# wg-perception/PartsBasedDetector

Hardware: AMD Instinct MI355X
Metric: detect() frames/sec, 640x480, 26-part person model (higher is better)
Workload: dtype f32

## Files before the change

partsbaseddetector_amd/csrc/k_hog.hip:

```cpp
#include "pbd_internal.hpp"
#include "pbd_split.hpp"

#ifdef PBD_PROBES
__device__ unsigned long long pbd_hog_dbg[8];
#define HOG_STAMP(i) do { if (blockIdx.x == 0 && threadIdx.x == 0) pbd_hog_dbg[i] = wall_clock64(); } while (0)
void hog_debug_read(unsigned long long* out) { hipMemcpyFromSymbol(out, HIP_SYMBOL(pbd_hog_dbg), sizeof(unsigned long long) * 8); }
#else
#define HOG_STAMP(i) do { } while (0)
void hog_debug_read(unsigned long long* out) { for (int i = 0; i < 8; ++i) out[i] = 0; }
#endif

#define HOG_LUT_SIDE 511
template <typename T>
__device__ __forceinline__ int hog_snap(T dx, T dy) {
  const T uu[9] = {1.000, 0.9397, 0.7660, 0.5000, 0.1736, -0.1736, -0.5000, -0.7660, -0.9397};
  const T vv[9] = {0.000, 0.3420, 0.6428, 0.8660, 0.9848, 0.9848, 0.8660, 0.6428, 0.3420};
  T best_dot = 0;
  int best_o = 0;
#pragma unroll
  for (int o = 0; o < 9; ++o) {
    T dot = uu[o] * dx + vv[o] * dy;
    if (dot > best_dot) { best_dot = dot; best_o = o; }
    else if (-dot > best_dot) { best_dot = -dot; best_o = o + 9; }
  }
  return best_o;
}
template <typename T>
__global__ __launch_bounds__(256) void k_hog_binlut(uint8_t* __restrict__ lut) {
  const int i = blockIdx.x * 256 + threadIdx.x;
  if (i >= HOG_LUT_SIDE * HOG_LUT_SIDE) return;
  const int iy = i / HOG_LUT_SIDE, ix = i - iy * HOG_LUT_SIDE;
  lut[i] = (uint8_t)hog_snap<T>((T)(ix - 255), (T)(iy - 255));
}
size_t hog_binlut_bytes() { return (size_t)HOG_LUT_SIDE * HOG_LUT_SIDE; }
void launch_hog_binlut(uint8_t* lut, int ts, hipStream_t s) {
  const int n = HOG_LUT_SIDE * HOG_LUT_SIDE;
  if (ts == 8) hipLaunchKernelGGL(k_hog_binlut<double>, dim3((n + 255) / 256), dim3(256), 0, s, lut);
  else hipLaunchKernelGGL(k_hog_binlut<float>, dim3((n + 255) / 256), dim3(256), 0, s, lut);
}

#define HOG_NT 384

template <typename T, int SBIN_T, int TC_T, typename IT = uint8_t>
__global__ __launch_bounds__(HOG_NT, 5) void k_hog(const HogTile* __restrict__ tiles, const LevelDev* __restrict__ levels,
                                                const uint8_t* __restrict__ pyr, T* __restrict__ feat, int cn,
                                                int sbin_rt, int tc_rt, const uint8_t* __restrict__ binlut, uint16_t* __restrict__ split, int split_parts) {
  const int sbin = SBIN_T > 0 ? SBIN_T : sbin_rt;
  const int tc = TC_T > 0 ? TC_T : tc_rt;
  extern __shared__ __attribute__((aligned(16))) char smem[];
#ifdef PBD_HOG_PRIO
  __builtin_amdgcn_s_setprio(PBD_HOG_PRIO);
#endif
  HOG_STAMP(0);
  const HogTile t = tiles[blockIdx.x];
  const LevelDev lv = levels[t.level];
  const int bpp = cn * (int)sizeof(IT);
  constexpr bool NEED_IP = !(SBIN_T > 0 && (SBIN_T & 1) == 0);
  const HogLds L = hog_lds_layout(sbin, tc, bpp, (int)sizeof(T), NEED_IP);
  T* mag = (T*)(smem + L.mag_off);
  uint8_t* bin = (uint8_t*)(smem + L.bin_off);
  uint8_t* raw = (uint8_t*)(smem + L.raw_off);
  T* hist = (T*)(smem + L.hist_off);
  T* norm = (T*)(smem + L.norm_off);
  T* ninv = (T*)(smem + L.ninv_off);
  T* wy0 = (T*)(smem + L.tab_off);
  T* wy1 = wy0 + L.PT;
  T* wx0 = wy1 + L.PT;
  T* wx1 = wx0 + L.PT;
  int* ipy = (int*)(wx1 + L.PT);
  int* ipx = ipy + L.PT;
  const int PT = L.PT, NB = L.NB, RT = L.RT, RP = L.RP, tid = threadIdx.x;
  const int w = lv.iw, h = lv.ih, bw = lv.bw, bh = lv.bh;
  const int vw = bw * sbin, vh = bh * sbin;
  const uint8_t* im = pyr + lv.img_off;
  const int stride = w * bpp;
  const int py0 = t.cy0 * sbin - (sbin + 1) / 2 - L.P0, px0 = t.cx0 * sbin - (sbin + 1) / 2 - L.P0;
  const int ry0 = py0 - L.MG, rx0 = px0 - L.MG;

  {
    const int wpr = RP >> 2;
    const int nword = RT * wpr;
    const int rowbytes = stride;
    const int b00 = rx0 * bpp;
    constexpr int LBW = 7;
    if (rowbytes >= 4) {
      const unsigned wmagic = 0xFFFFFFFFu / (unsigned)wpr + 1u;
      auto place = [&](int i, int& b0, int& la) {
        const int r = wpr > 1 ? (int)__umulhi((unsigned)i, wmagic) : i, k = i - r * wpr;
        b0 = b00 + 4 * k;
        la = r * RP + 4 * k;
        return min(max(ry0 + r, 0), h - 1);
      };
      for (int i0 = tid; i0 < nword; i0 += HOG_NT * LBW) {
        unsigned wv[LBW];
#pragma unroll
        for (int j = 0; j < LBW; ++j) {
          int b0, la;
          const int sy = place(min(i0 + j * HOG_NT, nword - 1), b0, la);
          wv[j] = *(const __attribute__((aligned(1))) unsigned*)(im + (size_t)sy * stride + min(max(b0, 0), rowbytes - 4));
        }
#pragma unroll
        for (int j = 0; j < LBW; ++j) {
          int b0, la;
          place(min(i0 + j * HOG_NT, nword - 1), b0, la);
          const int sh = min(max(b0, 0), rowbytes - 4) - b0;
          const int a8 = 8 * min(abs(sh), 3);
          *(unsigned*)(raw + la) = sh > 0 ? wv[j] << a8 : wv[j] >> a8;
        }
      }
    } else {
      for (int i = tid; i < nword; i += HOG_NT) {
        const int r = i / wpr, k = i - r * wpr;
        const int sy = min(max(ry0 + r, 0), h - 1);
        const int b0 = b00 + 4 * k;
        const uint8_t* src = im + (size_t)sy * stride;
        unsigned v = 0;
#pragma unroll
        for (int q = 0; q < 4; ++q) v |= (unsigned)src[min(max(b0 + q, 0), rowbytes - 1)] << (8 * q);
        *(unsigned*)(raw + r * RP + 4 * k) = v;
      }
    }
  }
  for (int i = tid; i < 2 * PT; i += HOG_NT) {
    const bool isx = i >= PT;
    const int j = isx ? i - PT : i;
    const int p = (isx ? px0 : py0) + j;
    T pp = (T)(((double)(T)p + 0.5) / (double)(T)sbin - 0.5);
    int ip = (int)t_floor(pp);
    T v0 = pp - (T)ip;
    T v1 = (T)(1.0 - (double)v0);
    if (isx) { wx0[j] = v0; wx1[j] = v1; if constexpr (NEED_IP) ipx[j] = ip; }
    else { wy0[j] = v0; wy1[j] = v1; if constexpr (NEED_IP) ipy[j] = ip; }
  }
  __syncthreads();
  HOG_STAMP(1);

  for (int i = tid; i < PT * PT; i += HOG_NT) {
    const int wy = i / PT, wx = i - wy * PT;
    const int y = py0 + wy, x = px0 + wx;
    T m = (T)0;
    int b = 0;
    if (y >= 1 && y < vh - 1 && x >= 1 && x < vw - 1) {
      const int sx = min(x, w - 2), sy = min(y, h - 2);
      if constexpr (sizeof(IT) > 1) {
        const IT* s = (const IT*)(raw + (sy - ry0) * RP + (sx - rx0) * bpp);
        const int rs = RP / (int)sizeof(IT);
        T dx, dy, v;
        if (cn == 1) {
          dy = (T)(s[rs] - s[-rs]);
          dx = (T)(s[1] - s[-1]);
          v = dx * dx + dy * dy;
        } else {
          const T dyb = (T)(s[rs] - s[-rs]), dxb = (T)(s[3] - s[-3]);
          const T vb = dxb * dxb + dyb * dyb;
          const T dyg = (T)(s[rs + 1] - s[-rs + 1]), dxg = (T)(s[4] - s[-2]);
          const T vg = dxg * dxg + dyg * dyg;
          dy = (T)(s[rs + 2] - s[-rs + 2]); dx = (T)(s[5] - s[-1]);
          v = dx * dx + dy * dy;
          if (vg > v) { v = vg; dx = dxg; dy = dyg; }
          if (vb > v) { v = vb; dx = dxb; dy = dyb; }
        }
        b = hog_snap<T>(dx, dy);
        m = t_sqrt(v);
      } else {
      const uint8_t* s = raw + (sy - ry0) * RP + (sx - rx0) * cn;
      int dxi, dyi, vi;
      if (cn == 1) {
        dyi = (int)s[RP] - (int)s[-RP];
        dxi = (int)s[1] - (int)s[-1];
      } else {
        const int dyb = (int)s[RP] - (int)s[-RP], dxb = (int)s[3] - (int)s[-3];
        const int dyg = (int)s[RP + 1] - (int)s[-RP + 1], dxg = (int)s[4] - (int)s[-2];
        dyi = (int)s[RP + 2] - (int)s[-RP + 2]; dxi = (int)s[5] - (int)s[-1];
        vi = dxi * dxi + dyi * dyi;
        const int vg = dxg * dxg + dyg * dyg, vb = dxb * dxb + dyb * dyb;
        if (vg > vi) { vi = vg; dxi = dxg; dyi = dyg; }
        if (vb > vi) { vi = vb; dxi = dxb; dyi = dyb; }
      }
      vi = dxi * dxi + dyi * dyi;
      b = binlut[(dyi + 255) * HOG_LUT_SIDE + (dxi + 255)];
      m = t_sqrt((T)vi);
      }
    }
    const int wq = wx / sbin, pi = wy * L.MP + (wx - wq * sbin) * L.QS + wq;
    mag[pi] = m;
    bin[pi] = (uint8_t)b;
  }
  __syncthreads();
  for (int i = tid; i < NB * NB * PBD_NORIENT; i += HOG_NT) hist[i] = (T)0;
  __syncthreads();
  HOG_STAMP(2);

  for (int bl = tid; bl < NB * NB; bl += HOG_NT) {
    const int lby = bl / NB, lbx = bl - lby * NB;
    const int by = t.cy0 + lby, bx = t.cx0 + lbx;
    if (by >= bh || bx >= bw) continue;
    T* hb = hist + bl;
    const int NBB = NB * NB;
    if constexpr (SBIN_T > 0 && (SBIN_T & 1) == 0) {
      const int wy_lo = lby * SBIN_T, wx_lo = lbx * SBIN_T;
      T fxv[2 * SBIN_T];
#pragma unroll
      for (int dx = 0; dx < 2 * SBIN_T; ++dx) fxv[dx] = dx < SBIN_T ? wx0[wx_lo + dx] : wx1[wx_lo + dx];
#pragma unroll 2
      for (int dy = 0; dy < 2 * SBIN_T; ++dy) {
        const int wy = wy_lo + dy;
        const T fy = dy < SBIN_T ? wy0[wy] : wy1[wy];
        const uint8_t* brow = bin + wy * L.MP + lbx;
        const T* mrow = mag + wy * L.MP + lbx;
#pragma unroll
        for (int dx = 0; dx < 2 * SBIN_T; ++dx) {
          const int pi = (dx % SBIN_T) * L.QS + dx / SBIN_T;
          hb[brow[pi] * NBB] += (fy * fxv[dx]) * mrow[pi];
        }
      }
    } else {
      const int wy_lo = lby * sbin, wx_lo = lbx * sbin, span = 2 * sbin + 2;
#pragma unroll 2
      for (int dy = 0; dy < span; ++dy) {
        const int wy = wy_lo + dy;
        if (wy >= PT) break;
        const int iy = ipy[wy];
        T fy;
        if (iy == by) fy = wy1[wy]; else if (iy == by - 1) fy = wy0[wy]; else continue;
        for (int dx = 0; dx < span; ++dx) {
          const int wx = wx_lo + dx;
          if (wx >= PT) break;
          const int ix = ipx[wx];
          T fx;
          if (ix == bx) fx = wx1[wx]; else if (ix == bx - 1) fx = wx0[wx]; else continue;
          const int wq = wx / sbin, pi = wy * L.MP + (wx - wq * sbin) * L.QS + wq;
          hb[bin[pi] * NBB] += (fy * fx) * mag[pi];
        }
      }
    }
  }
  __syncthreads();
  HOG_STAMP(3);

  for (int i = tid; i < NB * NB; i += HOG_NT) {
    const T* hsrc = hist + i;
    const int NBB = NB * NB;
    T acc = (T)0;
#pragma unroll
    for (int o = 0; o < 9; ++o) {
      T s = hsrc[o * NBB] + hsrc[(o + 9) * NBB];
      acc += s * s;
    }
    norm[i] = acc;
  }
  __syncthreads();

  const int NC = tc + 1;
  for (int i = tid; i < NC * NC; i += HOG_NT) {
    const int y = i / NC, x = i - y * NC;
    const T* p = norm + y * NB + x;
    T s = p[0] + p[1] + p[NB] + p[NB + 1];
    ninv[i] = (T)(1.0f / sqrt((double)s + 0.0001));
  }
  __syncthreads();

  HOG_STAMP(4);
  T* out = feat + lv.cell_off * PBD_FLEN;
  T* stg = (T*)(smem + L.out_off);
  const int ncell = tc * tc, half = (ncell + 1) / 2;
  for (int c0 = 0; c0 < ncell; c0 += half) {
    const int cell = c0 + tid;
    if (tid < half && cell < ncell) {
      const int ly = cell / tc, lx = cell - ly * tc;
      if (t.cy0 + ly < bh - 2 && t.cx0 + lx < bw - 2) {
        const T n1 = ninv[(ly + 1) * NC + lx + 1], n2 = ninv[ly * NC + lx + 1];
        const T n3 = ninv[(ly + 1) * NC + lx], n4 = ninv[ly * NC + lx];
        const T* hsrc = hist + ((ly + 1) * NB + lx + 1);
        const int NBB = NB * NB;
        T* d = stg + tid * (PBD_FLEN + 1);
        T t1 = 0, t2 = 0, t3 = 0, t4 = 0;
#pragma unroll 6
        for (int o = 0; o < PBD_NORIENT; ++o) {
          const T val = hsrc[o * NBB];
          const T h1 = t_fmin(val * n1, (T)0.2), h2 = t_fmin(val * n2, (T)0.2);
          const T h3 = t_fmin(val * n3, (T)0.2), h4 = t_fmin(val * n4, (T)0.2);
          d[o] = (T)(0.5 * (double)(h1 + h2 + h3 + h4));
          t1 += h1; t2 += h2; t3 += h3; t4 += h4;
        }
#pragma unroll 3
        for (int o = 0; o < PBD_NORIENT / 2; ++o) {
          const T sum = hsrc[o * NBB] + hsrc[(o + PBD_NORIENT / 2) * NBB];
          const T h1 = t_fmin(sum * n1, (T)0.2), h2 = t_fmin(sum * n2, (T)0.2);
          const T h3 = t_fmin(sum * n3, (T)0.2), h4 = t_fmin(sum * n4, (T)0.2);
          d[PBD_NORIENT + o] = (T)(0.5 * (double)(h1 + h2 + h3 + h4));
        }
        d[27] = (T)(0.2357 * (double)t1);
        d[28] = (T)(0.2357 * (double)t2);
        d[29] = (T)(0.2357 * (double)t3);
        d[30] = (T)(0.2357 * (double)t4);
        d[31] = (T)0;
      }
    }
    __syncthreads();
    for (int i = tid; i < half * PBD_FLEN; i += HOG_NT) {
      const int k = i & 31, lc = i >> 5;
      const int cl = c0 + lc;
      const int ly = cl / tc, lx = cl - ly * tc;
      const int cy = t.cy0 + ly, cx = t.cx0 + lx;
      if (cl < ncell && cy < bh - 2 && cx < bw - 2) {
        const T v = stg[lc * (PBD_FLEN + 1) + k];
        const size_t gc = (size_t)cy * lv.cw + cx;
        out[gc * PBD_FLEN + k] = v;
        if constexpr (sizeof(T) == 4) {
          if (split && split_parts == 3) {
            feat_split_bf16(v, split + (lv.cell_off + gc) * (3 * PBD_FLEN) + k, PBD_FLEN);
          } else if (split) {
            feat_split_f16(v, (_Float16*)split + (lv.cell_off + gc) * (2 * PBD_FLEN) + k, PBD_FLEN);
          }
        }
      }
    }
    __syncthreads();
  }
  HOG_STAMP(5);
}

template <typename T>
static void launch_hog_t(const HogTile* tiles, int ntiles, const LevelDev* levels, const uint8_t* pyr, T* feat,
                         int cn, int sbin, int tc, const uint8_t* binlut, uint16_t* split, int split_parts, int depth, hipStream_t s) {
  const int esz = depth == PBD_DEPTH_16U ? 2 : depth == PBD_DEPTH_32F ? 4 : depth == PBD_DEPTH_64F ? 8 : 1;
  auto go = [&](auto kern, bool need_ip) {
    const size_t lds = hog_lds_layout(sbin, tc, cn * esz, (int)sizeof(T), need_ip).total;
    static LdsOptIn optin;
    optin.ensure((const void*)kern, lds);
    hipLaunchKernelGGL(kern, dim3(ntiles), dim3(HOG_NT), lds, s, tiles, levels, pyr, feat, cn, sbin, tc, binlut, split, split_parts);
  };
  if (depth == PBD_DEPTH_16U) go(k_hog<T, 0, 0, uint16_t>, true);
  else if (depth == PBD_DEPTH_32F) go(k_hog<T, 0, 0, float>, true);
  else if (depth == PBD_DEPTH_64F) go(k_hog<T, 0, 0, double>, true);
  else if (sbin == 4 && tc == 16) go(k_hog<T, 4, 16>, false);
  else if (sbin == 4 && tc == 8) go(k_hog<T, 4, 8>, false);
  else if (sbin == 8 && tc == 8) go(k_hog<T, 8, 8>, false);
  else go(k_hog<T, 0, 0>, true);
}

void launch_hog(const HogTile* tiles, int ntiles, const LevelDev* levels, const uint8_t* pyr, void* feat, int ts,
                int cn, int sbin, int tc, const uint8_t* binlut, uint16_t* split, int split_parts, int depth, hipStream_t s) {
  if (ntiles <= 0) return;
  if (ts == 8) launch_hog_t<double>(tiles, ntiles, levels, pyr, (double*)feat, cn, sbin, tc, binlut, nullptr, 0, depth, s);
  else launch_hog_t<float>(tiles, ntiles, levels, pyr, (float*)feat, cn, sbin, tc, binlut, split, split_parts, depth, s);
}
```

partsbaseddetector_amd/csrc/pbd_lds.hpp:

```cpp
#pragma once
#include <stddef.h>
#include "pbd_plan.hpp"

#ifdef __HIPCC__
#define PBD_HD __host__ __device__ inline
#else
#define PBD_HD inline
#endif

#define DT_SEGS 72
PBD_HD size_t dt_hdr_bytes(int nt, int ts, int its, int lpb) {
  return ((size_t)lpb * 16 + DT_SEGS * 4 + (size_t)nt * (ts + 4 * its) + 15) & ~(size_t)15;
}
inline size_t dt_lds_bytes(int stride, int lpb, int ts, int nt) {
  const int its = stride <= 256 ? 1 : 2;
  return (size_t)lpb * stride * (2 * ts + its) + dt_hdr_bytes(nt, ts, its, lpb) + (((size_t)stride + 1) & ~(size_t)1) * 8 + 16;
}

struct HogLds {
  int PT;
  int NB;
  int P0;
  int MG;
  int RT;
  int RP;
  int QS;
  int MP;
  size_t mag_off, bin_off, hist_off, norm_off, ninv_off, tab_off, raw_off, out_off, total;
};

PBD_HD HogLds hog_lds_layout(int sbin, int tc, int bpp, int ts, bool need_ip = true) {
  HogLds L;
  L.NB = tc + 2;
  L.P0 = (sbin & 1) ? 1 : 0;
  L.PT = L.NB * sbin + sbin + 2 * L.P0;
  L.MG = sbin / 2 + 2;
  L.RT = L.PT + L.MG + 1;
  L.RP = (bpp & 7) ? (L.RT * bpp + 3) & ~3 : (L.RT * bpp + 7) & ~7;
  L.QS = (L.PT + sbin - 1) / sbin;
  L.MP = L.QS * sbin;
  size_t o = 0;
  const size_t nn = (size_t)ts * (L.NB * L.NB + (tc + 1) * (tc + 1));
  L.mag_off = o; L.norm_off = o; L.ninv_off = o + (size_t)ts * L.NB * L.NB;
  L.out_off = (o + nn + 15) & ~(size_t)15;
  {
    const size_t a = (size_t)ts * L.PT * L.MP, b = L.out_off + (size_t)ts * ((tc * tc + 1) / 2) * (PBD_FLEN + 1);
    o += ((a > b ? a : b) + 15) & ~(size_t)15;
  }
  const size_t hist_bytes = (size_t)ts * L.NB * L.NB * PBD_NORIENT, raw_bytes = (size_t)L.RT * L.RP;
  L.hist_off = o; L.raw_off = o;
  o += ((hist_bytes > raw_bytes ? hist_bytes : raw_bytes) + 15) & ~(size_t)15;
  L.tab_off = o; o += ((size_t)ts * 2 + (need_ip ? sizeof(int) : 0)) * 2 * L.PT;
  L.bin_off = (o + 3) & ~(size_t)3; o = L.bin_off + (size_t)L.PT * L.MP;
  L.total = (o + 15) & ~(size_t)15;
  return L;
}
inline size_t hog_lds_bytes(int sbin, int tc, int ts, int bpp = 3) { return hog_lds_layout(sbin, tc, bpp, ts).total; }
```

Measured before the change: 2415.

## Pack HOG magnitude and bin into one LDS word and split normalization roles

For even fixed sbin with uint8 input and float output, gradient magnitude and orientation bin are packed into a single 32-bit LDS word, with the bin in the top bits and the magnitude rescaled to fit the remaining bits. This removes the separate bin array and halves the LDS reads in the histogram loop. Interpolation weights become compile-time constants, so the weight tables are no longer built or stored. The normalization step splits each cell's work across three lane groups, and feature stores are widened to two elements per store. These changes shrink LDS use and per-thread work, at the risk of precision loss for very small or denormal magnitudes and of a mismatched LDS size on the host side, since the host computes the packed flag using sbin=4 even for the sbin=8 variant.

```diff
diff --git a/partsbaseddetector_amd/csrc/hog_pack.hpp b/partsbaseddetector_amd/csrc/hog_pack.hpp
--- /dev/null
+++ b/partsbaseddetector_amd/csrc/hog_pack.hpp
@@ -0,0 +1,45 @@
+#pragma once
+#include <stdint.h>
+#include <type_traits>
+
+#ifdef __HIPCC__
+#define HOG_PACK_HD __host__ __device__ inline
+#else
+#define HOG_PACK_HD inline
+#endif
+
+template <typename T, int SBIN, typename IT> constexpr bool hog_packed() {
+  return std::is_same<T, float>::value && std::is_same<IT, uint8_t>::value && SBIN > 0 && (SBIN & 1) == 0;
+}
+
+HOG_PACK_HD uint32_t hog_f2u(float f) { uint32_t u; __builtin_memcpy(&u, &f, 4); return u; }
+HOG_PACK_HD float hog_u2f(uint32_t u) { float f; __builtin_memcpy(&f, &u, 4); return f; }
+
+HOG_PACK_HD uint32_t hog_pack_bits(uint32_t bits, uint32_t bin) {
+  const uint32_t e = bits >> 23, e4 = e ? e - 126u : 0u;
+  return bin << 27 | e4 << 23 | (bits & 0x7FFFFFu);
+}
+HOG_PACK_HD uint32_t hog_unpack_bits(uint32_t w) {
+  const uint32_t t = w & 0x07FFFFFFu;
+  return t ? t + (126u << 23) : 0u;
+}
+HOG_PACK_HD uint32_t hog_unpack_bin(uint32_t w) { return w >> 27; }
+
+HOG_PACK_HD uint32_t hog_pack(float g, uint32_t bin) { return bin << 27 | hog_f2u(g * 0x1p-126f); }
+HOG_PACK_HD float hog_unpack_scaled(uint32_t w) { return hog_u2f(w & 0x07FFFFFFu); }
+#define HOG_UNSCALE 0x1p126f
+
+template <typename T, int SBIN> struct HogWeights;
+template <typename T> struct HogWeights<T, 4> {
+  static constexpr T w0[4] = {(T)0.625, (T)0.875, (T)0.125, (T)0.375};
+  static constexpr T w1[4] = {(T)0.375, (T)0.125, (T)0.875, (T)0.625};
+};
+template <typename T> struct HogWeights<T, 8> {
+  static constexpr T w0[8] = {(T)0.5625, (T)0.6875, (T)0.8125, (T)0.9375, (T)0.0625, (T)0.1875, (T)0.3125, (T)0.4375};
+  static constexpr T w1[8] = {(T)0.4375, (T)0.3125, (T)0.1875, (T)0.0625, (T)0.9375, (T)0.8125, (T)0.6875, (T)0.5625};
+};
+template <typename T, int SBIN> HOG_PACK_HD constexpr T hog_w0(int p) { return HogWeights<T, SBIN>::w0[((p % SBIN) + SBIN) % SBIN]; }
+template <typename T, int SBIN> HOG_PACK_HD constexpr T hog_w1(int p) { return HogWeights<T, SBIN>::w1[((p % SBIN) + SBIN) % SBIN]; }
+template <typename T, int SBIN> HOG_PACK_HD constexpr T hog_footprint_weight(int d) {
+  return d < SBIN ? hog_w0<T, SBIN>(d + SBIN / 2) : hog_w1<T, SBIN>(d + SBIN / 2);
+}
diff --git a/partsbaseddetector_amd/csrc/k_hog.hip b/partsbaseddetector_amd/csrc/k_hog.hip
--- a/partsbaseddetector_amd/csrc/k_hog.hip
+++ b/partsbaseddetector_amd/csrc/k_hog.hip
@@ -1,5 +1,6 @@
 #include "pbd_internal.hpp"
 #include "pbd_split.hpp"
+#include "hog_pack.hpp"
 
 #ifdef PBD_PROBES
 __device__ unsigned long long pbd_hog_dbg[8];
@@ -56,8 +57,10 @@
   const LevelDev lv = levels[t.level];
   const int bpp = cn * (int)sizeof(IT);
   constexpr bool NEED_IP = !(SBIN_T > 0 && (SBIN_T & 1) == 0);
-  const HogLds L = hog_lds_layout(sbin, tc, bpp, (int)sizeof(T), NEED_IP);
+  constexpr bool PACKED = hog_packed<T, SBIN_T, IT>();
+  const HogLds L = hog_lds_layout(sbin, tc, bpp, (int)sizeof(T), NEED_IP, PACKED);
   T* mag = (T*)(smem + L.mag_off);
+  unsigned* pk = (unsigned*)(smem + L.mag_off);
   uint8_t* bin = (uint8_t*)(smem + L.bin_off);
   uint8_t* raw = (uint8_t*)(smem + L.raw_off);
   T* hist = (T*)(smem + L.hist_off);
@@ -121,16 +124,18 @@
       }
     }
   }
-  for (int i = tid; i < 2 * PT; i += HOG_NT) {
-    const bool isx = i >= PT;
-    const int j = isx ? i - PT : i;
-    const int p = (isx ? px0 : py0) + j;
-    T pp = (T)(((double)(T)p + 0.5) / (double)(T)sbin - 0.5);
-    int ip = (int)t_floor(pp);
-    T v0 = pp - (T)ip;
-    T v1 = (T)(1.0 - (double)v0);
-    if (isx) { wx0[j] = v0; wx1[j] = v1; if constexpr (NEED_IP) ipx[j] = ip; }
-    else { wy0[j] = v0; wy1[j] = v1; if constexpr (NEED_IP) ipy[j] = ip; }
+  if constexpr (NEED_IP) {
+    for (int i = tid; i < 2 * PT; i += HOG_NT) {
+      const bool isx = i >= PT;
+      const int j = isx ? i - PT : i;
+      const int p = (isx ? px0 : py0) + j;
+      T pp = (T)(((double)(T)p + 0.5) / (double)(T)sbin - 0.5);
+      int ip = (int)t_floor(pp);
+      T v0 = pp - (T)ip;
+      T v1 = (T)(1.0 - (double)v0);
+      if (isx) { wx0[j] = v0; wx1[j] = v1; ipx[j] = ip; }
+      else { wy0[j] = v0; wy1[j] = v1; ipy[j] = ip; }
+    }
   }
   __syncthreads();
   HOG_STAMP(1);
@@ -183,8 +188,8 @@
       }
     }
     const int wq = wx / sbin, pi = wy * L.MP + (wx - wq * sbin) * L.QS + wq;
-    mag[pi] = m;
-    bin[pi] = (uint8_t)b;
+    if constexpr (PACKED) pk[pi] = hog_pack(m, (unsigned)b);
+    else { mag[pi] = m; bin[pi] = (uint8_t)b; }
   }
   __syncthreads();
   for (int i = tid; i < NB * NB * PBD_NORIENT; i += HOG_NT) hist[i] = (T)0;
@@ -198,21 +203,25 @@
     T* hb = hist + bl;
     const int NBB = NB * NB;
     if constexpr (SBIN_T > 0 && (SBIN_T & 1) == 0) {
-      const int wy_lo = lby * SBIN_T, wx_lo = lbx * SBIN_T;
-      T fxv[2 * SBIN_T];
-#pragma unroll
-      for (int dx = 0; dx < 2 * SBIN_T; ++dx) fxv[dx] = dx < SBIN_T ? wx0[wx_lo + dx] : wx1[wx_lo + dx];
-#pragma unroll 2
+      const int wy_lo = lby * SBIN_T;
+#pragma unroll
       for (int dy = 0; dy < 2 * SBIN_T; ++dy) {
         const int wy = wy_lo + dy;
-        const T fy = dy < SBIN_T ? wy0[wy] : wy1[wy];
+        const T fy = hog_footprint_weight<T, SBIN_T>(dy);
         const uint8_t* brow = bin + wy * L.MP + lbx;
         const T* mrow = mag + wy * L.MP + lbx;
+        const unsigned* prow = pk + wy * L.MP + lbx;
 #pragma unroll
         for (int dx = 0; dx < 2 * SBIN_T; ++dx) {
           const int pi = (dx % SBIN_T) * L.QS + dx / SBIN_T;
-          hb[brow[pi] * NBB] += (fy * fxv[dx]) * mrow[pi];
-        }
+          if constexpr (PACKED) {
+            const unsigned wv = prow[pi];
+            hb[hog_unpack_bin(wv) * NBB] += (T)((fy * hog_footprint_weight<T, SBIN_T>(dx)) * HOG_UNSCALE) * (T)hog_unpack_scaled(wv);
+          } else {
+            hb[brow[pi] * NBB] += (fy * hog_footprint_weight<T, SBIN_T>(dx)) * mrow[pi];
+          }
+        }
+        if constexpr (PACKED) __builtin_amdgcn_sched_barrier(0);
       }
     } else {
       const int wy_lo = lby * sbin, wx_lo = lbx * sbin, span = 2 * sbin + 2;
@@ -264,54 +273,80 @@
   T* out = feat + lv.cell_off * PBD_FLEN;
   T* stg = (T*)(smem + L.out_off);
   const int ncell = tc * tc, half = (ncell + 1) / 2;
+  constexpr int RS = TC_T > 0 ? ((TC_T * TC_T + 1) / 2 < 64 ? 64 : (TC_T * TC_T + 1) / 2) : HOG_NT;
+  static_assert(TC_T == 0 || 3 * RS <= HOG_NT, "three lane roles per cell must fit the workgroup");
   for (int c0 = 0; c0 < ncell; c0 += half) {
-    const int cell = c0 + tid;
-    if (tid < half && cell < ncell) {
+    const int role = TC_T > 0 ? tid / RS : 0, lc = tid - role * RS;
+    const int cell = c0 + lc;
+    if (lc < half && cell < ncell && role < 3) {
       const int ly = cell / tc, lx = cell - ly * tc;
       if (t.cy0 + ly < bh - 2 && t.cx0 + lx < bw - 2) {
         const T n1 = ninv[(ly + 1) * NC + lx + 1], n2 = ninv[ly * NC + lx + 1];
         const T n3 = ninv[(ly + 1) * NC + lx], n4 = ninv[ly * NC + lx];
         const T* hsrc = hist + ((ly + 1) * NB + lx + 1);
         const int NBB = NB * NB;
-        T* d = stg + tid * (PBD_FLEN + 1);
-        T t1 = 0, t2 = 0, t3 = 0, t4 = 0;
+        T* d = stg + lc * (PBD_FLEN + 1);
+        if (role == 0) {
+          T t1 = 0, t2 = 0, t3 = 0, t4 = 0;
 #pragma unroll 6
-        for (int o = 0; o < PBD_NORIENT; ++o) {
-          const T val = hsrc[o * NBB];
-          const T h1 = t_fmin(val * n1, (T)0.2), h2 = t_fmin(val * n2, (T)0.2);
-          const T h3 = t_fmin(val * n3, (T)0.2), h4 = t_fmin(val * n4, (T)0.2);
-          d[o] = (T)(0.5 * (double)(h1 + h2 + h3 + h4));
-          t1 += h1; t2 += h2; t3 += h3; t4 += h4;
-        }
-#pragma unroll 3
-        for (int o = 0; o < PBD_NORIENT / 2; ++o) {
-          const T sum = hsrc[o * NBB] + hsrc[(o + PBD_NORIENT / 2) * NBB];
-          const T h1 = t_fmin(sum * n1, (T)0.2), h2 = t_fmin(sum * n2, (T)0.2);
-          const T h3 = t_fmin(sum * n3, (T)0.2), h4 = t_fmin(sum * n4, (T)0.2);
-          d[PBD_NORIENT + o] = (T)(0.5 * (double)(h1 + h2 + h3 + h4));
-        }
-        d[27] = (T)(0.2357 * (double)t1);
-        d[28] = (T)(0.2357 * (double)t2);
-        d[29] = (T)(0.2357 * (double)t3);
-        d[30] = (T)(0.2357 * (double)t4);
-        d[31] = (T)0;
+          for (int o = 0; o < PBD_NORIENT; ++o) {
+            const T val = hsrc[o * NBB];
+            const T h1 = t_fmin(val * n1, (T)0.2), h2 = t_fmin(val * n2, (T)0.2);
+            const T h3 = t_fmin(val * n3, (T)0.2), h4 = t_fmin(val * n4, (T)0.2);
+            d[o] = (T)(0.5 * (double)(h1 + h2 + h3 + h4));
+            t1 += h1; t2 += h2; t3 += h3; t4 += h4;
+          }
+          d[27] = (T)(0.2357 * (double)t1);
+          d[28] = (T)(0.2357 * (double)t2);
+          d[29] = (T)(0.2357 * (double)t3);
+          d[30] = (T)(0.2357 * (double)t4);
+          d[31] = (T)0;
+        }
+        const int o0 = TC_T > 0 ? (role == 1 ? 0 : 5) : 0, o1 = TC_T > 0 ? (role == 1 ? 5 : PBD_NORIENT / 2) : PBD_NORIENT / 2;
+        if (TC_T == 0 || role > 0) {
+          for (int o = o0; o < o1; ++o) {
+            const T sum = hsrc[o * NBB] + hsrc[(o + PBD_NORIENT / 2) * NBB];
+            const T h1 = t_fmin(sum * n1, (T)0.2), h2 = t_fmin(sum * n2, (T)0.2);
+            const T h3 = t_fmin(sum * n3, (T)0.2), h4 = t_fmin(sum * n4, (T)0.2);
+            d[PBD_NORIENT + o] = (T)(0.5 * (double)(h1 + h2 + h3 + h4));
+          }
+        }
       }
     }
     __syncthreads();
-    for (int i = tid; i < half * PBD_FLEN; i += HOG_NT) {
-      const int k = i & 31, lc = i >> 5;
+    constexpr int VK = 2;
+    struct alignas(VK * sizeof(T) < 16 ? VK * sizeof(T) : 16) FeatV { T a[VK]; };
+    for (int i = tid; i < half * (PBD_FLEN / VK); i += HOG_NT) {
+      const int k = (i & (PBD_FLEN / VK - 1)) * VK, lc = i / (PBD_FLEN / VK);
       const int cl = c0 + lc;
       const int ly = cl / tc, lx = cl - ly * tc;
       const int cy = t.cy0 + ly, cx = t.cx0 + lx;
       if (cl < ncell && cy < bh - 2 && cx < bw - 2) {
-        const T v = stg[lc * (PBD_FLEN + 1) + k];
+        FeatV v;
+#pragma unroll
+        for (int j = 0; j < VK; ++j) v.a[j] = stg[lc * (PBD_FLEN + 1) + k + j];
         const size_t gc = (size_t)cy * lv.cw + cx;
-        out[gc * PBD_FLEN + k] = v;
+        *(FeatV*)(out + gc * PBD_FLEN + k) = v;
         if constexpr (sizeof(T) == 4) {
           if (split && split_parts == 3) {
-            feat_split_bf16(v, split + (lv.cell_off + gc) * (3 * PBD_FLEN) + k, PBD_FLEN);
+            uint16_t p[3][VK];
+#pragma unroll
+            for (int j = 0; j < VK; ++j) feat_split_bf16(v.a[j], &p[0][j], VK);
+            uint16_t* sp = split + (lv.cell_off + gc) * (3 * PBD_FLEN) + k;
+#pragma unroll
+            for (int q = 0; q < 3; ++q)
+              *(unsigned*)(sp + q * PBD_FLEN) = (unsigned)p[q][0] | (unsigned)p[q][1] << 16;
           } else if (split) {
-            feat_split_f16(v, (_Float16*)split + (lv.cell_off + gc) * (2 * PBD_FLEN) + k, PBD_FLEN);
+            _Float16 p[2][VK];
+#pragma unroll
+            for (int j = 0; j < VK; ++j) feat_split_f16(v.a[j], &p[0][j], VK);
+            _Float16* sp = (_Float16*)split + (lv.cell_off + gc) * (2 * PBD_FLEN) + k;
+#pragma unroll
+            for (int q = 0; q < 2; ++q) {
+              unsigned w;
+              __builtin_memcpy(&w, p[q], sizeof(w));
+              *(unsigned*)(sp + q * PBD_FLEN) = w;
+            }
           }
         }
       }
@@ -326,7 +361,8 @@
                          int cn, int sbin, int tc, const uint8_t* binlut, uint16_t* split, int split_parts, int depth, hipStream_t s) {
   const int esz = depth == PBD_DEPTH_16U ? 2 : depth == PBD_DEPTH_32F ? 4 : depth == PBD_DEPTH_64F ? 8 : 1;
   auto go = [&](auto kern, bool need_ip) {
-    const size_t lds = hog_lds_layout(sbin, tc, cn * esz, (int)sizeof(T), need_ip).total;
+    const bool packed = !need_ip && hog_packed<T, 4, uint8_t>();
+    const size_t lds = hog_lds_layout(sbin, tc, cn * esz, (int)sizeof(T), need_ip, packed).total;
     static LdsOptIn optin;
     optin.ensure((const void*)kern, lds);
     hipLaunchKernelGGL(kern, dim3(ntiles), dim3(HOG_NT), lds, s, tiles, levels, pyr, feat, cn, sbin, tc, binlut, split, split_parts);
diff --git a/partsbaseddetector_amd/csrc/pbd_lds.hpp b/partsbaseddetector_amd/csrc/pbd_lds.hpp
--- a/partsbaseddetector_amd/csrc/pbd_lds.hpp
+++ b/partsbaseddetector_amd/csrc/pbd_lds.hpp
@@ -29,7 +29,7 @@
   size_t mag_off, bin_off, hist_off, norm_off, ninv_off, tab_off, raw_off, out_off, total;
 };
 
-PBD_HD HogLds hog_lds_layout(int sbin, int tc, int bpp, int ts, bool need_ip = true) {
+PBD_HD HogLds hog_lds_layout(int sbin, int tc, int bpp, int ts, bool need_ip = true, bool packed = false) {
   HogLds L;
   L.NB = tc + 2;
   L.P0 = (sbin & 1) ? 1 : 0;
@@ -50,8 +50,8 @@
   const size_t hist_bytes = (size_t)ts * L.NB * L.NB * PBD_NORIENT, raw_bytes = (size_t)L.RT * L.RP;
   L.hist_off = o; L.raw_off = o;
   o += ((hist_bytes > raw_bytes ? hist_bytes : raw_bytes) + 15) & ~(size_t)15;
-  L.tab_off = o; o += ((size_t)ts * 2 + (need_ip ? sizeof(int) : 0)) * 2 * L.PT;
-  L.bin_off = (o + 3) & ~(size_t)3; o = L.bin_off + (size_t)L.PT * L.MP;
+  L.tab_off = o; if (need_ip) o += ((size_t)ts * 2 + sizeof(int)) * 2 * L.PT;
+  L.bin_off = (o + 3) & ~(size_t)3; if (!packed) o = L.bin_off + (size_t)L.PT * L.MP;
   L.total = (o + 15) & ~(size_t)15;
   return L;
 }
```

Measured after the change: 2441 (median of 6 runs). No clear change (+1.1%).
